# status-im/nim-blscurve

Hardware: AMD Instinct MI355X
Metric: BLS sig verifications/sec (batch) (higher is better)
Workload: dtype int64

## Files before the change

nim-blscurve_amd/csrc/host_api.inc:

```
#pragma once
#include "plan.hpp"
#include "devres.hpp"
using plan::SIG_SLOTS_MAX;
namespace cols = plan::cols;
static_assert(plan::WAVE == (uint32_t)WAVE && plan::N_LINES == (uint32_t)N_LINES, "plan.hpp restates the wave size and the Miller loop's step count");
static_assert(plan::FP_WORDS == (uint32_t)FPW && plan::G1_WORDS == (uint32_t)G1W && plan::G2_WORDS == (uint32_t)G2W && plan::F12_WORDS == (uint32_t)F12W,
              "plan.hpp restates the words of an element in device buffers");

struct msm_ws {
    dev_buf<uint8_t> d_pts, d_sc;
    dev_buf<uint32_t> pts_int;
    dev_buf<uint32_t> hist, offs, cursor, sorted, order, chist, winout, out, part, shist;
    dev_event ev_fork, ev_bucketed, ev_g[2], ev_tail[2];
    dev_buf<uint4> buckets, segout;
};
struct msm_many_ws {
    dev_buf<uint8_t> d_pts, d_sc;
    dev_buf<uint32_t> pts_int, offs_dev, hist, offs, cursor, order, chist, sorted, part, out;
    dev_buf<uint4> buckets, segout;
};
struct ptab_ws {
    dev_buf<uint32_t> scratch, hist, offs, cursor, order, chist, sorted, part, out;
    dev_buf<uint4> buckets, segout;
    uint32_t last_plan[3] = {0, 0, 0};
// ... 517 lines not shown
    }
    if (hi > B) hi = (uint32_t)B;
    size_t base = n_total / B, rem = n_total % B;
    auto off = [&](size_t c) { return c < rem ? (base + 1) * c : base * c + rem; };
    *first = off(lo);
    *count = off(hi) - off(lo);
}

static void host_sha256_32(const uint32_t (&in)[8], uint32_t (&out)[8]) {
    uint32_t w[16] = {in[0], in[1], in[2], in[3], in[4], in[5], in[6], in[7], 0x80000000u, 0, 0, 0, 0, 0, 0, 256};
    sha256_init(out);
    sha256_compress_core(out, w);
}
static void host_serial_chain(const uint8_t rnd[32], size_t n, uint64_t* out) {
    uint32_t seed[8], nx[8];
    for (int i = 0; i < 8; i++) nx[i] = ((uint32_t)rnd[4 * i] << 24) | ((uint32_t)rnd[4 * i + 1] << 16) | ((uint32_t)rnd[4 * i + 2] << 8) | rnd[4 * i + 3];
    host_sha256_32(nx, seed);
    for (size_t j = 0; j < n; j++) {
        uint64_t r;
        do {
            host_sha256_32(seed, nx);
            for (int i = 0; i < 8; i++) seed[i] = nx[i];
            r = digest_low_u64_le(seed);
        } while (r == 0);
        out[j] = r;
    }
}
static void host_combine_chain(const uint8_t rnd[32], size_t n, uint64_t* out) {
    uint32_t seed[8], nx[8];
    for (int i = 0; i < 8; i++) seed[i] = ((uint32_t)rnd[4 * i] << 24) | ((uint32_t)rnd[4 * i + 1] << 16) | ((uint32_t)rnd[4 * i + 2] << 8) | rnd[4 * i + 3];
    int avail = 0;
    for (size_t i = 0; i < n; i++) {
        for (;;) {
            if (avail == 0) {
                host_sha256_32(seed, nx);
                for (int j = 0; j < 8; j++) seed[j] = nx[j];
                avail = 4;
            }
            avail--;
            uint64_t w = (uint64_t)bswap32(seed[2 * avail]) | ((uint64_t)bswap32(seed[2 * avail + 1]) << 32);
            if (w != 0) {
                out[i] = w;
                break;
            }
        }
    }
}

static inline void launch_k_tail(const mi355_bls_ctx* c, hipStream_t st, const uint32_t* L, uint32_t* states, uint32_t kk, int mode, uint32_t* gt_out,
                                 uint32_t* verdict, uint32_t sstride, int blob) {
    if (c->coop) k_tail_rows<<<1, K_TAIL_THREADS, 0, st>>>(L, states, kk, mode, gt_out, verdict, sstride, blob);
    else k_tail<<<1, TAIL_THREADS, 0, st>>>(L, states, kk, mode, gt_out, verdict, sstride, blob);
}
static void launch_lines_at(const pair_store& ps, const plan::stage& t, uint32_t first, uint32_t count, hipStream_t st) {
    if (!t.team) {
        k_lines<<<t.grid, WAVE, 0, st>>>(ps.P, ps.H, first, count, ps.stride, ps.lines);
        return;
    }
    switch (t.form) {
        case plan::TEAM_ROWS: k_team_lines_rows<<<t.grid, 256, 0, st>>>(ps.P, ps.H, first, count, ps.stride, ps.lines); break;
        case plan::TEAM_ROWS2: k_team_lines_rows2<<<t.grid, 256, 0, st>>>(ps.P, ps.H, first, count, ps.stride, ps.lines); break;
        case plan::TEAM_SPREAD: k_team_lines_spread<<<t.grid, WAVE, 0, st>>>(ps.P, ps.H, first, count, ps.stride, ps.lines); break;
        case plan::TEAM_WIDE: k_team_lines<<<t.grid, WAVE, 0, st>>>(ps.P, ps.H, first, count, ps.stride, ps.lines); break;
    }
}
static void launch_lines(const pair_store& ps, const plan::lines_plan& p, hipStream_t st) {
    launch_lines_at(ps, p.main, 0, p.main_pairs, st);
    if (p.extra_pairs) launch_lines_at(ps, p.extra, p.main_pairs, p.extra_pairs, st);
}

static int enqueue_line_products(mi355_bls_ctx* c, const pair_store& ps, uint32_t npairs, hipStream_t st, hipEvent_t mid_ev) {
    c->fold_form = (c->coop || c->alone) ? 1 : 0;
    const plan::lineprod_plan p = plan::lineprod_for(c->slots, c->nblk_cap, ps.stride, npairs, c->fold_form != 0);
    k_lineprod<<<dim3(N_LINES, p.nblk), WAVE, 0, st>>>(ps.lines, npairs, ps.stride, p.m, c->d_lpart, p.nblk, p.per_lane);
    if (mid_ev) HIPCHK(hipEventRecord(mid_ev, st));
    if (c->fold_form) {
        uint32_t* mid = c->d_lpart + plan::lpart_mid_words(c->nblk_cap);
        k_fold<<<dim3(N_LINES, p.nb1), TAIL_THREADS, 0, st>>>(c->d_lpart, p.nblk * WAVE, p.per, p.live - (p.nb1 - 1) * p.per, p.nb1 > 1 ? mid : c->d_L);
        if (p.nb1 > 1) k_fold<<<dim3(N_LINES, 1), TAIL_THREADS, 0, st>>>(mid, p.nb1, p.nb1, p.nb1, c->d_L);
    } else {
        k_lineprod2<<<N_LINES, WAVE, 0, st>>>(c->d_lpart, p.nblk * WAVE, c->d_L);
    }
    return 0;
}

static int run_pairs(mi355_bls_ctx* c, const uint8_t* d_sets, size_t n, hipStream_t st, bool pop = false);
static int run_slice(mi355_bls_ctx* c, mi355_bls_ctx* p, const uint8_t* d_sets, size_t n_total, uint32_t nchunks, uint32_t chunk_lo, uint32_t chunk_cnt,
                     size_t tuple_base, size_t n, int serial, size_t serial_off, uint32_t slice, hipStream_t st, hipEvent_t blind_done, bool pop = false) {
    HIPCHK(hipEventRecord(c->ev[0], st));
    if (serial) {
        HIPCHK(hipMemcpyAsync(c->d_r, p->h_r.data() + serial_off, n * 8, hipMemcpyHostToDevice, st));
    } else {
        k_blind<<<plan::waves_for(chunk_cnt), WAVE, 0, st>>>(p->d_rnd, n_total, nchunks, chunk_lo, chunk_cnt, tuple_base, n, p->d_carry + 8 * (slice & 1),
                                                                p->d_carry + 8 * ((slice + 1) & 1), c->d_r);
    }
    if (blind_done) HIPCHK(hipEventRecord(blind_done, st));
    return run_pairs(c, d_sets, n, st, pop);
}
static int run_pairs(mi355_bls_ctx* c, const uint8_t* d_sets, size_t n, hipStream_t st, bool pop) {
    const uint32_t n32 = (uint32_t)n;
    const pair_store ps = c->batch_pairs();
    HIPCHK(hipEventRecord(c->ev[1], st));
    const plan::slice_plan p = plan::slice_for(c->slots, c->coop, c->coop && ensure_side(c), n);
    const uint32_t nb = p.nb, cw = p.cw, nwin = p.nwin, total = p.total;
    const bool fork = p.side == plan::SIDE_FORK, fork_sig = p.side == plan::SIDE_FORK_SIG;
    const auto stream_of = [&](plan::stream_role r) { return r == plan::STREAM_CALLER ? st : r == plan::STREAM_SIDE2 && c->side2 ? c->side2 : c->side; };
    hipStream_t sd = stream_of(p.pk_stream);
    hipStream_t ss = stream_of(p.sig_stream);
    if (fork || fork_sig) HIPCHK(hipStreamWaitEvent(c->side, c->ev[1], 0));
    if (fork && sd != c->side) HIPCHK(hipStreamWaitEvent(sd, c->ev[1], 0));
    launch_hash_map(c, d_sets, n32, st, pop);
    HIPCHK(hipEventRecord(c->ev_hm, st));
    launch_hash_clear(c, ps, n32, st);
    HIPCHK(hipEventRecord(c->ev[2], st));
    if (p.pkmul_spread) k_pkmul_spread<<<nb, WAVE, 0, sd>>>(d_sets, n32, c->d_r, ps.P, ps.stride, c->d_flags, c->d_pktab);
    else k_pkmul<<<nb, WAVE, 0, sd>>>(d_sets, n32, c->d_r, ps.P, ps.stride, c->d_flags, c->d_pktab);
    HIPCHK(hipEventRecord(c->ev[3], sd));
    {
        msm_win W{nwin, cw, 0};
        uint32_t *hist = c->d_sig_hist, *offs = hist + SIG_SLOTS_MAX, *cursor = offs + SIG_SLOTS_MAX;
        HIPCHK(hipEventRecord(c->ev_s0, ss));
        HIPCHK(hipMemsetAsync(hist, 0, (size_t)total * 4, ss));
        k_sig_convert<<<nb, WAVE, 0, ss>>>(d_sets, n32, c->d_sig_pts);
        k_msm_hist<<<dim3(nb, nwin), WAVE, 0, ss>>>(reinterpret_cast<const uint8_t*>(c->d_r.p), 8, n32, W, cw, hist);
        k_msm_scan<<<nwin, WAVE, 0, ss>>>(hist, cw, offs, cursor);
        k_msm_scatter<<<dim3(nb, nwin), WAVE, 0, ss>>>(reinterpret_cast<const uint8_t*>(c->d_r.p), 8, n32, W, cw, cursor, c->d_sig_sorted);
        k_sig_bucket<<<p.bucket_grid, WAVE, 0, ss>>>(c->d_sig_pts, c->d_sig_sorted, offs, hist, n32, cw, p.lshift, total,
                                                     c->d_sig_consts + (cw == 8 ? (size_t)SIG_SLOTS_MAX * G1W : 0), ps.H, ps.P, ps.stride, (size_t)n32);
        c->sig_c = cw;
        c->sig_slots = total;
        c->agg_valid = false;
    }
    uint32_t npairs = n32 + total;
    if (p.extra_apart) launch_lines_at(ps, p.extra_lines, n32, total, ss);
    HIPCHK(hipEventRecord(c->ev[4], ss));
    if (fork) {
        HIPCHK(hipStreamWaitEvent(st, c->ev[4], 0));
        HIPCHK(hipStreamWaitEvent(st, c->ev[3], 0));
    }
    HIPCHK(hipEventRecord(c->ev_l0, st));
    launch_lines(ps, p.lines, st);
    if (fork_sig) HIPCHK(hipStreamWaitEvent(st, c->ev[4], 0));
    HIPCHK(hipEventRecord(c->ev[5], st));
    {
        int rcp = enqueue_line_products(c, ps, npairs, st, c->ev_lp);
        if (rcp) return rcp;
    }
    c->wide_recorded = true;
    HIPCHK(hipEventRecord(c->ev[6], st));
    launch_k_tail(c, st, c->d_L, c->d_states, 1, 1, c->d_gt, c->d_flags + 1, 144, 0);
    HIPCHK(hipEventRecord(c->ev[7], st));
    HIPCHK(hipGetLastError());
    c->last_n = n;
    c->have_gt = false;
    c->gt_is_fv = false;
    return 0;
}

static int ensure_lanes(mi355_bls_ctx* c, int want) {
    for (dev_event* e : {&c->ev_sl0, &c->ev_blind[0], &c->ev_blind[1], &c->ev_blind[2]})
        if (!*e)
            if (int rc = e->create(hipEventDisableTiming)) return rc;
    int have = 0;
    for (int k = 0; k < want && k < 2; k++) {
        if (c->lane[k]) {
            have = k + 1;
            continue;
        }
        mi355_bls_ctx* raw = nullptr;
        dev_stream s;
        dev_event e;
        if (mi355_bls_ctx_create(&raw, c->device, c->cap) != 0) raw = nullptr;
        std::unique_ptr<mi355_bls_ctx> x(raw);
        if (!x || !s.create() || e.create(hipEventDisableTiming) != 0) {
            x.reset();
            (void)hipGetLastError();
            (void)hipSetDevice(c->device);
            break;
        }
        x->is_lane = true;
        x->coop = false;
        c->lane_st[k] = std::move(s);
        c->lane_ev[k] = std::move(e);
        c->lane[k] = std::move(x);
        have = k + 1;
    }
    return have;
}
static int run_shard(mi355_bls_ctx* c, const uint8_t* src_dev, const uint8_t* src_host, size_t n_total, uint32_t nchunks, uint32_t chunk_lo, uint32_t chunk_cnt,
                     size_t tuple_base, size_t n, int serial, const uint8_t rnd[32], hipStream_t st, bool pop = false, const uint64_t* chosen_r = nullptr) {
    (void)chunk_lo; (void)chunk_cnt;
    HIPCHK(hipSetDevice(c->device));
    if (c->fail_next_enqueue) {
        c->fail_next_enqueue = false;
// ... 3755 lines not shown
```

nim-blscurve_amd/csrc/kernels.hip:

```cpp
#include <hip/hip_runtime.h>

#include <algorithm>
#include <atomic>
#include <chrono>
#include <cstdio>
#include <cstdlib>
#include <cstring>
#include <mutex>
#include <string>
#include <unordered_map>
#include <vector>

#include "../../include/blscurve_mi355x.h"
#include "deser.hpp"
#include "h2c.hpp"
#include "pairing.hpp"
#include "vereach.hpp"
#include "aggveach.hpp"
#include "aggsets.hpp"
#include "aggbits.hpp"
#include "combsets.hpp"
#include "manyeach.hpp"
#include "pairprod.hpp"
#include "bymsg.hpp"
// ... 748 lines not shown
#endif
}
__global__ void __launch_bounds__(256) __attribute__((amdgpu_waves_per_eu(1, 1)))
k_team_lines_rows(const uint4* __restrict__ P, const uint4* __restrict__ H, uint32_t first, uint32_t count, size_t stride, uint4* __restrict__ lines) {
    team_lines_rows_body(P, H, first, count, stride, lines);
}
__global__ void __launch_bounds__(256) __attribute__((amdgpu_waves_per_eu(2, 2)))
k_team_lines_rows2(const uint4* __restrict__ P, const uint4* __restrict__ H, uint32_t first, uint32_t count, size_t stride, uint4* __restrict__ lines) {
    team_lines_rows_body(P, H, first, count, stride, lines);
}

#if defined(__HIP_DEVICE_COMPILE__)
#include "../build/pkmul_asm.inc"
__device__ __forceinline__ uint32_t pkmul_asm(uint64_t r, uint8_t* table, uint32_t off16, uint4* P, uint32_t pstride16, uint32_t lds) {
    uint32_t flag;
    asm volatile(BLS_PKMUL_ASM_BODY : "=v"(flag) : "v"((uint32_t)r), "v"((uint32_t)(r >> 32)), "s"(table), "s"(0u), "v"(off16), "s"(P), "s"(pstride16), "s"(lds) : BLS_PKMUL_ASM_CLOBBERS);
    return flag;
}
#endif
__device__ __forceinline__ void pkmul_body(const uint8_t* __restrict__ sets, uint32_t n, const uint64_t* __restrict__ r, uint4* __restrict__ P,
                                           size_t stride, uint32_t* __restrict__ flags, uint8_t* __restrict__ table) {
    uint32_t i = blockIdx.x * blockDim.x + threadIdx.x;
    if (i >= n) return;
    const uint32_t* w = reinterpret_cast<const uint32_t*>(sets + (size_t)i * 320);
    g1_aff pk = ld_g1a_blst(w);
    const bool inf = aff_is_inf(pk);
    if (inf) atomicOr(flags, 1u);
#if defined(__HIP_DEVICE_COMPILE__)
    if (table) {
        __shared__ bls_u32x4 key_slot[BLS_LDS_SLOT];
        if (inf) {
            soa_st_g1(P, stride, i, jac_inf<fp>());
        } else {
            fp2_lds_put((bls_lds_u32x4*)key_slot, fp2{pk.x, pk.y});
            if (pkmul_asm(r[i], table, i * 16u, P, (uint32_t)(stride * 16), (uint32_t)(uintptr_t)(bls_lds_u32x4*)key_slot))
                soa_st_g1(P, stride, i, jac_mul_u64_w4_body(pk, r[i]));
        }
        return;
    }
#endif
    g1_jac q = jac_mul_u64_w4_body(pk, r[i]);
    soa_st_g1(P, stride, i, q);
}
__global__ void __launch_bounds__(WAVE, 2) k_pkmul(const uint8_t* __restrict__ sets, uint32_t n, const uint64_t* __restrict__ r, uint4* __restrict__ P,
                                                   size_t stride, uint32_t* __restrict__ flags, uint8_t* __restrict__ table) {
    pkmul_body(sets, n, r, P, stride, flags, table);
}
__global__ void __launch_bounds__(WAVE) __attribute__((amdgpu_waves_per_eu(1, 1)))
k_pkmul_spread(const uint8_t* __restrict__ sets, uint32_t n, const uint64_t* __restrict__ r, uint4* __restrict__ P, size_t stride, uint32_t* __restrict__ flags,
               uint8_t* __restrict__ table) {
    pkmul_body(sets, n, r, P, stride, flags, table);
}

#if defined(__HIP_DEVICE_COMPILE__)
#include "../build/lines_asm.inc"
__device__ __forceinline__ void lines_asm(uint4* lines, uint32_t stride16, uint32_t off16, uint32_t skip, uint32_t lds_a, uint32_t lds_b) {
    asm volatile(BLS_LINES_ASM_BODY : : "s"(lines), "s"(stride16), "v"(off16), "v"(skip), "s"(lds_a), "s"(lds_b) : BLS_LINES_ASM_CLOBBERS);
}
#endif
__global__ void __launch_bounds__(WAVE) k_lines(const uint4* __restrict__ P, const uint4* __restrict__ H, uint32_t first, uint32_t count, size_t stride,
                                                uint4* __restrict__ lines) {
    uint32_t i = blockIdx.x * blockDim.x + threadIdx.x;
    if (i >= count) return;
    i += first;
    g1_jac p = soa_ld_g1(P, stride, i);
    g2_jac q = soa_ld_g2(H, stride, i);
#if defined(__HIP_DEVICE_COMPILE__)
    if (stride * 16 * 24 < ((size_t)1 << 32)) {
        __shared__ bls_u32x4 hand_over[4 * BLS_LDS_SLOT];
        const bool skip = jac_is_inf(p) | jac_is_inf(q);
        if (skip) {
            const line_t one = line_one();
            for (int s = 0; s < N_LINES; s++) {
                uint4* b = lines + (size_t)s * 24 * stride;
                soa_st2(b, stride, 0, i, one.l0);
                soa_st2(b, stride, 2, i, one.l1);
                soa_st2(b, stride, 4, i, one.l2);
            }
        }
        const g1_pre pre = g1_precompute(p);
        g2_proj t = g2_to_proj(q);
        bls_lds_u32x4* ho = (bls_lds_u32x4*)hand_over;
        fp2_lds_put(ho, fp2_reduce(t.x));
        fp2_lds_put(ho + BLS_LDS_SLOT, fp2_reduce(t.y));
        fp2_lds_put(ho + 2 * BLS_LDS_SLOT, fp2_reduce(t.z));
        fp2_lds_put(ho + 3 * BLS_LDS_SLOT, fp2{pre.z3, pre.nxz3});
        fp2_lds_put((bls_lds_u32x4*)bls_xchg, fp2{pre.xz, pre.y});
        lines_asm(lines, (uint32_t)(stride * 16), i * 16u, skip ? 1u : 0u, (uint32_t)(uintptr_t)ho, (uint32_t)(uintptr_t)(bls_lds_u32x4*)bls_xchg);
        return;
    }
#endif
    miller_lines(p, q, [&](int s, const line_t& l) {
        uint4* b = lines + (size_t)s * 24 * stride;
        soa_st2(b, stride, 0, i, l.l0);
        soa_st2(b, stride, 2, i, l.l1);
        soa_st2(b, stride, 4, i, l.l2);
    });
}

#if defined(__HIP_DEVICE_COMPILE__)
#include "../build/lineprod_asm.inc"
__device__ __forceinline__ void lineprod_asm(const uint4* step_base, uint32_t stride16, uint32_t npairs, uint32_t first, uint32_t rounds, uint32_t* out,
                                             uint32_t lds_buf) {
    asm volatile(BLS_LINEPROD_ASM_BODY : : "s"(step_base), "s"(stride16), "s"(npairs), "s"(first), "s"(rounds), "s"(out), "s"(lds_buf) : BLS_LINEPROD_ASM_CLOBBERS);
}
#endif
__global__ void __launch_bounds__(WAVE) k_lineprod(const uint4* __restrict__ lines, uint32_t npairs, size_t stride, uint32_t m,
                                                   uint32_t* __restrict__ part, uint32_t nblk, int per_lane) {
    uint32_t s = blockIdx.x, b = blockIdx.y;
    const uint4* base = lines + (size_t)s * 24 * stride;
    size_t first = (size_t)b * WAVE * m;
#if defined(__HIP_DEVICE_COMPILE__)
    __shared__ bls_u32x4 line_slots[4 * BLS_LDS_SLOT];
#endif
#if defined(__HIP_DEVICE_COMPILE__)
    if (per_lane == 1) {
        uint32_t rounds = 0;
        if (first < npairs) {
            size_t left = (npairs - first + WAVE - 1) / WAVE;
            rounds = left < m ? (uint32_t)left : m;
        }
        lineprod_asm(base, (uint32_t)(stride * 16), npairs, (uint32_t)first, rounds, part + ((size_t)s * nblk + b) * WAVE * F12W,
                     (uint32_t)(uintptr_t)(bls_lds_u32x4*)line_slots);
        return;
    }
#endif
    auto ld_line = [&](size_t j0) {
        size_t i = j0 + threadIdx.x;
        bool v = i < npairs;
        size_t ia = v ? i : j0;
        line_t l{soa_ld2(base, stride, 0, ia), soa_ld2(base, stride, 2, ia), soa_ld2(base, stride, 4, ia)};
        return line_t{fp2_select(v, l.l0, fp2_one()), fp2_select(v, l.l1, fp2_zero()), fp2_select(v, l.l2, fp2_zero())};
    };
    fp12 f = fp12_one();
#if defined(__HIP_DEVICE_COMPILE__)
    line_ops_lds lops{(bls_lds_u32x4*)line_slots};
#else
    line_ops_lds lops{};
#endif
    if (first < npairs) {
        f = fp12_from_line(ld_line(first));
#pragma clang loop unroll(disable)
        for (uint32_t j = 1; j < m; j++) {
            size_t j0 = first + (size_t)j * WAVE;
            if (j0 >= npairs) break;
// ... 1090 lines not shown
}
__global__ void __launch_bounds__(WAVE) k_ptab_scatter(const uint8_t* __restrict__ sc, fixed_addr A, pip_win W, uint32_t* __restrict__ cursor, uint32_t* __restrict__ sorted) {
    const uint32_t p = blockIdx.x * WAVE + threadIdx.x, w = blockIdx.y;
    if (p >= A.pairs) return;
    const int32_t d = pipm_digit(sc, p, W, w);
    if (d) {
        const uint32_t j = fixed_owner(A, p);
        const uint32_t pos = atomicAdd(&cursor[fixed_bucket(A, j, w, (uint32_t)(d < 0 ? -d : d))], 1u);
        sorted[pos] = fixed_entry(A, w, fixed_point(A, p, j)) | (d < 0 ? 0x80000000u : 0u);
    }
}
__global__ void __launch_bounds__(WAVE) k_debug_ptab_rows(const uint32_t* __restrict__ tab, uint32_t n, uint32_t w0, uint32_t nw, uint32_t i0, uint32_t ni,
                                                          uint32_t* __restrict__ out) {
    const uint32_t t = blockIdx.x * WAVE + threadIdx.x;
    if (t >= nw * ni) return;
    const uint32_t w = w0 + t / ni, i = i0 + t % ni;
    const uint32_t* e = tab + ((size_t)w * n + i) * (2 * FPW);
    uint32_t* o = out + (size_t)t * 24;
    if (e[FP_N]) {
        for (int q = 0; q < 24; q++) o[q] = 0;
    } else {
        st_fp_blst(o, ld_fp_int(e));
        st_fp_blst(o + 12, ld_fp_int(e + FPW));
    }
}

__device__ __forceinline__ g1_jac ld_jac_blst(const uint32_t* w, const g1_jac*) { return ld_g1_blst(w); }
__device__ __forceinline__ g2_jac ld_jac_blst(const uint32_t* w, const g2_jac*) { return ld_g2_blst(w); }
template <class F>
__global__ void __launch_bounds__(WAVE) k_jac_sum_blst(const uint32_t* __restrict__ parts, uint32_t k, uint32_t stride, uint32_t* __restrict__ out) {
    jac<F> acc = jac_inf<F>();
    for (uint32_t j = threadIdx.x; j < k; j += WAVE) acc = padd(acc, ld_jac_blst(parts + (size_t)j * stride, (const jac<F>*)nullptr));
    int top = 32;
    while (top >= 1 && (uint32_t)top >= k) top >>= 1;
    for (int d = top; d >= 1; d >>= 1) {
        jac<F> o = shfl_down_struct(acc, d);
        acc = padd(acc, o);
    }
    if (threadIdx.x == 0) st_jac_blst(out, acc);
}

__global__ void __launch_bounds__(WAVE) k_sig_convert(const uint8_t* __restrict__ sets, uint32_t n, uint32_t* __restrict__ pts_int) {
    uint32_t i = blockIdx.x * WAVE + threadIdx.x;
    if (i >= n) return;
    g2_aff q = ld_g2a_blst(reinterpret_cast<const uint32_t*>(sets + (size_t)i * 320 + 128));
    uint32_t* o = pts_int + (size_t)i * 4 * FPW;
    st_fp_int(o, q.x.c0); st_fp_int(o + FPW, q.x.c1); st_fp_int(o + 2 * FPW, q.y.c0); st_fp_int(o + 3 * FPW, q.y.c1);
}
__global__ void __launch_bounds__(WAVE) k_sig_consts(uint32_t c, uint32_t total, uint32_t* __restrict__ out) {
    uint32_t g = blockIdx.x * WAVE + threadIdx.x;
    if (g >= total) return;
    uint64_t sc = (uint64_t)(g & ((1u << c) - 1u)) << (c * (g >> c));
    g1_aff ng{fp_from_const(k::G1_X), fp_from_const(k::G1_NEG_Y)};
    st_g1_int(out + (size_t)g * G1W, jac_mul_u64(ng, sc));
}
__global__ void __launch_bounds__(WAVE) k_sig_bucket(const uint32_t* __restrict__ pts, const uint32_t* __restrict__ sorted, const uint32_t* __restrict__ offs,
                                                     const uint32_t* __restrict__ hist, uint32_t n, uint32_t c, uint32_t lshift, uint32_t total,
                                                     const uint32_t* __restrict__ consts, uint4* __restrict__ H, uint4* __restrict__ P, size_t stride, size_t base) {
    uint32_t t = blockIdx.x * WAVE + threadIdx.x;
    uint32_t L = 1u << lshift, g = t >> lshift, s = t & (L - 1);
    xyzz<fp2> part = xyzz_inf<fp2>();
    if (g < total) {
        uint32_t w = g >> c, cnt = hist[g], off = offs[g];
        const uint32_t* srt = sorted + (size_t)w * n + off;
        for (uint32_t j = s; j < cnt; j += L) {
            const uint32_t* pw = pts + (size_t)srt[j] * (4 * FPW);
            g2_aff q{fp2{ld_fp_int(pw), ld_fp_int(pw + FPW)}, fp2{ld_fp_int(pw + 2 * FPW), ld_fp_int(pw + 3 * FPW)}};
            part = xyzz_add_aff(part, q);
        }
    }
    g2_jac acc = jac_from_xyzz(part);
    for (uint32_t d = L >> 1; d >= 1; d >>= 1) {
        g2_jac o = shfl_down_struct(acc, (int)d);
        acc = jac_add(acc, o);
    }
    if (g < total && s == 0) {
        soa_st_g2(H, stride, base + g, acc);
        soa_st_g1(P, stride, base + g, ld_g1_int(consts + (size_t)g * G1W));
    }
}
__global__ void __launch_bounds__(WAVE) k_sig_fold(const uint4* __restrict__ H, size_t stride, uint32_t n, uint32_t nwin, uint32_t c, uint32_t* __restrict__ agg_out) {
    __shared__ uint32_t wsum[32 * G2W];
    uint32_t w = threadIdx.x;
    if (w < nwin) {
        g2_jac S = jac_inf<fp2>(), T = jac_inf<fp2>();
        for (uint32_t d = (1u << c) - 1; d >= 1; d--) {
            S = jac_add(S, soa_ld_g2(H, stride, (size_t)n + ((w << c) | d)));
            T = jac_add(T, S);
        }
        st_g2_int(wsum + (size_t)w * G2W, T);
    }
    __syncthreads();
    if (threadIdx.x == 0) {
        g2_jac acc = ld_g2_int(wsum + (size_t)(nwin - 1) * G2W);
        for (uint32_t j = nwin - 1; j-- > 0;) {
            for (uint32_t i = 0; i < c; i++) acc = jac_dbl(acc);
            acc = jac_add(acc, ld_g2_int(wsum + (size_t)j * G2W));
        }
        st_g2_blst(agg_out, acc);
    }
}

__global__ void __launch_bounds__(WAVE) k_deser(const uint8_t* __restrict__ pks, const uint8_t* __restrict__ msgs, const uint8_t* __restrict__ sigs,
                                                uint32_t n, uint32_t dflags, uint8_t* __restrict__ sets, uint8_t* __restrict__ status,
                                                uint32_t* __restrict__ flags) {
    uint32_t i = blockIdx.x * WAVE + threadIdx.x;
    if (i >= n) return;
// ... 897 lines not shown
```

nim-blscurve_amd/csrc/pairing.hpp:

```cpp
#pragma once
#include "curve.hpp"
#include "tower.hpp"

namespace bls {

constexpr int N_LINES = 68;

struct g1_pre {
    fp z3, xz, nxz3, y;
};

BLS_HD g1_pre g1_precompute(const g1_jac& p) {
    fp z2 = fp_sqr(p.z);
    fp xz = fp_mul(p.x, p.z);
    return g1_pre{fp_mul(z2, p.z), xz, fp_neg(fp_carry(fp_add_nc(fp_dbl_nc(xz), xz))), p.y};
}

BLS_HD line_t line_one() { return line_t{fp2_one(), fp2_zero(), fp2_zero()}; }

using g2_proj = g2_jac;

BLS_HD g2_proj g2_to_proj(const g2_jac& q) {
    fp2 z2 = fp2_sqr(q.z);
    return g2_proj{fp2_mul(q.x, q.z), q.y, fp2_mul(z2, q.z)};
}

BLS_MID fp2 fp2_sqr_minus_12sqr(const fp2& a, const fp2& e) {
    const fp e4s = fp_dbl_nc(fp_carry(fp_dbl_nc(fp_add_nc(e.c0, e.c1))));
    const fp ed = fp_sub_pos(e.c0, e.c1);
    const fp e3d = fp_carry(fp_add_nc(fp_dbl_nc(ed), ed));
    const fp e8 = fp_dbl_nc(fp_carry(fp_dbl_nc(fp_dbl_nc(e.c0))));
    const fp e3 = fp_carry(fp_add_nc(fp_dbl_nc(e.c1), e.c1));
    return fp2{fp_dot2(fp_add_nc(a.c0, a.c1), fp_sub_nc(a.c0, a.c1), fp_neg(e4s), e3d), fp_dot2(fp_dbl_nc(a.c0), a.c1, fp_neg(e8), e3)};
}
template <class M>
BLS_MID line_t miller_dbl_step_m(g2_proj& t, const g1_pre& p, const M& m) {
    fp2 B = m.sqr(t.y);
    fp2 C = m.sqr(t.z);
    fp2 X2 = m.sqr(t.x);
    fp2 C4 = fp2_dbl_nc(fp2_carry(fp2_dbl_nc(fp2_mul_xi_nc(C))));
    fp2 E = fp2_reduce(fp2_add_nc(fp2_dbl_nc(C4), C4));
    fp2 F = fp2_add_nc(fp2_dbl_nc(E), E);
    fp2 H = fp2_carry(fp2_sub_nc(fp2_sub_nc(m.sqr(fp2_add(t.y, t.z)), B), C));
    fp2 XY2 = fp2_carry(fp2_sub_nc(fp2_sub_nc(m.sqr(fp2_add(t.x, t.y)), X2), B));
    fp2 x3 = m.mul(XY2, fp2_carry(fp2_sub_nc(B, F)));
    fp2 y3 = fp2_sqr_minus_12sqr(fp2_carry(fp2_add_nc(B, F)), E);
    fp2 z3 = fp2_carry(fp2_dbl_nc(fp2_dbl_nc(m.mul(B, H))));
    t = g2_proj{x3, y3, z3};
    fp2 BE = fp2_sub_nc(B, E);
    return line_t{fp2{m.mul(BE.c0, p.z3), m.mul(BE.c1, p.z3)}, fp2{m.mul(X2.c0, p.nxz3), m.mul(X2.c1, p.nxz3)}, fp2{m.mul(H.c0, p.y), m.mul(H.c1, p.y)}};
}
BLS_MID line_t miller_dbl_step(g2_proj& t, const g1_pre& p) { return miller_dbl_step_m(t, p, mul_shared{}); }

BLS_MID line_t miller_add_step(g2_proj& t, const g2_proj& q, const g1_pre& p) {
    fp2 Y1Z2 = fp2_mul(t.y, q.z), X1Z2 = fp2_mul(t.x, q.z), Z1Z2 = fp2_mul(t.z, q.z);
    fp2 u = fp2_sub(fp2_mul(q.y, t.z), Y1Z2);
    fp2 v = fp2_sub(fp2_mul(q.x, t.z), X1Z2);
    fp2 uu = fp2_sqr(u), vv = fp2_sqr(v);
    fp2 vvv = fp2_mul(v, vv);
    fp2 R = fp2_mul(vv, X1Z2);
    fp2 A = fp2_carry(fp2_sub_nc(fp2_sub_nc(fp2_mul(uu, Z1Z2), vvv), fp2_dbl_nc(R)));
    fp2 x3 = fp2_mul(v, A);
    fp2 y3 = fp2_reduce(fp2_sub_nc(fp2_mul(u, fp2_sub_nc(R, A)), fp2_mul(vvv, Y1Z2)));
    fp2 z3 = fp2_mul(vvv, Z1Z2);
    fp2 c0 = fp2_carry(fp2_sub_nc(fp2_mul(u, q.x), fp2_mul(v, q.y)));
    fp2 c1 = fp2_mul(u, q.z);
    fp2 c2 = fp2_mul(v, q.z);
    t = g2_proj{x3, y3, z3};
    return line_t{fp2_mul_fp(c0, p.z3), fp2_neg(fp2_mul_fp(c1, p.xz)), fp2_mul_fp(c2, p.y)};
}

template <class Sink>
BLS_HD void miller_lines(const g1_jac& pj, const g2_jac& qj, Sink&& sink) {
    bool skip = jac_is_inf(pj) | jac_is_inf(qj);
    g1_pre p = g1_precompute(pj);
    g2_proj q = g2_to_proj(qj);
    q = g2_proj{fp2_reduce(q.x), fp2_reduce(q.y), fp2_reduce(q.z)};
    g2_proj t = q;
    int s = 0;
    uint64_t rest = k::X_ABS & ~(1ull << 63);
    int pos = 63;
#pragma clang loop unroll(disable)
    while (pos > 0) {
        const int next = rest ? 63 - __builtin_clzll(rest) : 0;
        int n = pos - next;
#pragma clang loop unroll(disable)
        do {
            line_t l = miller_dbl_step(t, p);
            sink(s++, skip ? line_one() : l);
        } while (--n > 0);
        if (rest) {
            line_t a = miller_add_step(t, q, p);
            sink(s++, skip ? line_one() : a);
            rest &= ~(1ull << next);
        }
        pos = next;
    }
}

template <class Src>
BLS_HD fp12 miller_combine(Src&& src) {
    fp12 f = fp12_one();
    int s = 0;
    for (int bit = 62; bit >= 0; bit--) {
        f = fp12_sqr(f);
        f = fp12_mul(f, src(s++));
        if ((k::X_ABS >> bit) & 1) f = fp12_mul(f, src(s++));
    }
    return fp12_conj(f);
}

BLS_HDN fp12 fp12_cyc_exp_x(const fp12& a) {
    fp12 r = a;
    for (int bit = 62; bit >= 0; bit--) {
        r = fp12_sqr(r);
        if ((k::X_ABS >> bit) & 1) r = fp12_mul(r, a);
    }
    return fp12_conj(r);
}

BLS_HDN fp12 final_exp(const fp12& f) {
    fp12 t = fp12_mul(fp12_conj(f), fp12_inv(f));
    t = fp12_mul(fp12_frob2(t), t);
    fp12 a = fp12_mul(fp12_cyc_exp_x(t), fp12_conj(t));
    a = fp12_mul(fp12_cyc_exp_x(a), fp12_conj(a));
    fp12 b = fp12_mul(fp12_cyc_exp_x(a), fp12_frob(a));
    fp12 c = fp12_mul(fp12_mul(fp12_cyc_exp_x(fp12_cyc_exp_x(b)), fp12_frob2(b)), fp12_conj(b));
    return fp12_mul(c, fp12_mul(fp12_sqr(t), t));
}

}
```

nim-blscurve_amd/csrc/plan.hpp:

```cpp
#ifndef BLS_PLAN_HPP
#define BLS_PLAN_HPP
#include <cstddef>
#include <cstdint>

namespace plan {

constexpr uint32_t WAVE = 64;
constexpr uint32_t N_LINES = 68;
constexpr uint32_t FP_WORDS = 16;
constexpr uint32_t G1_WORDS = 3 * FP_WORDS, G2_WORDS = 6 * FP_WORDS, F12_WORDS = 12 * FP_WORDS;
constexpr uint32_t SIG_SLOTS_MAX = 2048;
static_assert(((64u / 8) << 8) == SIG_SLOTS_MAX, "the buckets of the 8-bit digits");
constexpr size_t SIG_WIDE_MIN = 40000;
constexpr uint32_t FORK_ITEMS_PER_SLOT = 16;

constexpr uint32_t TEAM_CLEAR_ITEMS_PER_SLOT = 11, TEAM_LINES_ITEMS_PER_SLOT = 18;
inline uint32_t team_clear_max(uint32_t slots) { return slots * TEAM_CLEAR_ITEMS_PER_SLOT; }
inline uint32_t team_lines_max(uint32_t slots) { return slots * TEAM_LINES_ITEMS_PER_SLOT; }

inline uint32_t waves_for(uint32_t count) { return (count + WAVE - 1) / WAVE; }
constexpr uint32_t GATHER_THREADS = 256;
inline uint32_t gather_blocks_for(size_t count) { return (uint32_t)((count + GATHER_THREADS - 1) / GATHER_THREADS); }

enum team_form { TEAM_ROWS, TEAM_ROWS2, TEAM_SPREAD, TEAM_WIDE };
// ... 19 lines not shown
enum hash_map_form { HASH_MAP_ROWS, HASH_MAP_SPREAD, HASH_MAP_PLAIN };
struct hash_map_plan {
    hash_map_form form;
    uint32_t grid;
};
inline hash_map_plan hash_map_for(uint32_t slots, bool coop, uint32_t n32) {
    const uint32_t waves = (2 * n32 + WAVE - 1) / WAVE;
    if (coop && (2 * n32 + 3) / 4 <= slots - slots / 8) return {HASH_MAP_ROWS, (2 * n32 + 3) / 4};
    if (coop && waves <= slots) return {HASH_MAP_SPREAD, waves};
    return {HASH_MAP_PLAIN, waves};
}

constexpr size_t POP_MAX_KEYS = (size_t)1 << 30;
constexpr uint32_t POP_RECORD_THREADS = 256;
inline uint32_t pop_records_grid(size_t n) { return (uint32_t)((n * 80 + POP_RECORD_THREADS - 1) / POP_RECORD_THREADS); }

constexpr uint8_t ADMIT_BAD_PROOF = 8;
inline size_t admit_survivors(const uint8_t* key_st, const uint8_t* proof_st, size_t n, uint32_t* list) {
    size_t m = 0;
    for (size_t i = 0; i < n; i++)
        if (key_st[i] == 0 && proof_st[i] == 0) list[m++] = (uint32_t)i;
    return m;
}
inline size_t admit_merge(const uint8_t* key_st, const uint8_t* proof_st, size_t n, const uint32_t* list, const uint8_t* verdicts, size_t m, uint8_t* status,
                          uint32_t* zero) {
    for (size_t i = 0; i < n; i++) status[i] = key_st[i] ? key_st[i] : proof_st[i];
    for (size_t j = 0; j < m; j++)
        if (verdicts[j] != 1) status[list[j]] = ADMIT_BAD_PROOF;
    size_t nz = 0;
    for (size_t i = 0; i < n; i++)
        if (status[i] != 0 && key_st[i] == 0) zero[nz++] = (uint32_t)i;
    return nz;
}

inline stage clear_for(uint32_t slots, bool coop, uint32_t n32) {
    return coop && n32 <= team_clear_max(slots) ? team_stage(slots, n32) : one_lane_stage(n32);
}

struct lines_plan {
    uint32_t main_pairs;
    stage main;
    uint32_t extra_pairs;
    stage extra;
};
inline lines_plan lines_for(uint32_t slots, bool coop, uint32_t npairs, uint32_t extra) {
    if (coop && npairs <= team_lines_max(slots)) return {npairs, team_stage(slots, npairs), 0, {}};
    if (coop && extra && extra < npairs && extra <= team_lines_max(slots) &&
        (npairs + WAVE - 1) / WAVE > slots * (((npairs - extra + WAVE - 1) / WAVE + slots - 1) / slots)) {
        const uint32_t main_pairs = npairs - extra;
        return {main_pairs, one_lane_stage(main_pairs), extra, team_stage(slots, extra)};
    }
    return {npairs, one_lane_stage(npairs), 0, {}};
}

enum side_mode { SIDE_NONE, SIDE_FORK, SIDE_FORK_SIG };
inline bool pkmul_spread_for(uint32_t slots, bool coop, uint32_t n) { return coop && waves_for(n) <= slots; }
enum stream_role { STREAM_CALLER, STREAM_SIDE, STREAM_SIDE2 };
struct slice_plan {
    uint32_t nb;
    hash_map_plan hash_map;
    stage clear;
    bool pkmul_spread;
    side_mode side;
    stream_role pk_stream, sig_stream;
    uint32_t cw, nwin, total;
    uint32_t lshift, bucket_grid;
    bool extra_apart;
    stage extra_lines;
    lines_plan lines;
};
inline slice_plan slice_for(uint32_t slots, bool coop, bool have_side, size_t n) {
    slice_plan p{};
    const uint32_t n32 = (uint32_t)n;
    p.nb = waves_for(n32);
    const bool fork = have_side && n32 <= FORK_ITEMS_PER_SLOT * slots;
    const bool fork_sig = !fork && have_side;
    p.side = fork ? SIDE_FORK : fork_sig ? SIDE_FORK_SIG : SIDE_NONE;
    p.pk_stream = fork ? STREAM_SIDE2 : STREAM_CALLER;
    p.sig_stream = (fork || fork_sig) ? STREAM_SIDE : STREAM_CALLER;
    p.hash_map = hash_map_for(slots, coop, n32);
    p.clear = clear_for(slots, coop, n32);
    p.pkmul_spread = pkmul_spread_for(slots, coop, n32);
    p.cw = n >= SIG_WIDE_MIN ? 8 : 4, p.nwin = 64 / p.cw, p.total = p.nwin << p.cw;
    uint32_t per = n32 >> p.cw, lshift = 0;
    const uint32_t per_lane_min = coop ? 16u : 64u;
    while (lshift < 6 && (per >> (lshift + 1)) >= per_lane_min) lshift++;
    while (lshift < 6 && ((p.total << (lshift + 1)) <= 16 * slots) && (per >> (lshift + 1)) >= 2) lshift++;
    p.lshift = lshift;
    p.bucket_grid = ((p.total << lshift) + WAVE - 1) / WAVE;
    p.extra_apart = fork_sig || (fork && p.total <= team_lines_max(slots));
    p.extra_lines = p.total <= team_lines_max(slots) ? team_stage(slots, p.total) : one_lane_stage(p.total);
    p.lines = p.extra_apart ? lines_for(slots, coop, n32, 0) : lines_for(slots, coop, n32 + p.total, p.total);
    return p;
}

struct lineprod_plan {
    uint32_t nblk, m;
    int per_lane;
    uint32_t live, per, nb1;
};
inline lineprod_plan lineprod_for(uint32_t slots, uint32_t nblk_cap, uint32_t stride, uint32_t npairs, bool fold) {
    lineprod_plan p{};
    uint32_t nblk = slots / N_LINES;
    if (nblk < 1) nblk = 1;
    if (nblk > nblk_cap) nblk = nblk_cap;
    uint32_t m = (npairs + WAVE * nblk - 1) / (WAVE * nblk);
    if (m < 1) m = 1;
    nblk = (npairs + WAVE * m - 1) / (WAVE * m);
    p.nblk = nblk, p.m = m;
    p.per_lane = (uint64_t)stride * 16 * 24 + (uint64_t)npairs * 16 < (1ull << 32) ? 1 : 2;
    if (fold) {
        size_t first_last = (size_t)(nblk - 1) * WAVE * m;
        p.live = (nblk - 1) * WAVE + (npairs - first_last < WAVE ? (uint32_t)(npairs - first_last) : WAVE);
        p.per = 1;
        while (p.per * p.per < p.live) p.per++;
        p.nb1 = (p.live + p.per - 1) / p.per;
    }
    return p;
}

constexpr uint32_t LINEPROD_RANGES_MAX = 64, FOLD_MID_ROOM = 64;
constexpr uint32_t SUM_G2_PARTS_MAX = 2048;
constexpr size_t SUM_PARTS_BYTES = 2048 * 2 * G1_WORDS * 4;
static_assert((size_t)SUM_G2_PARTS_MAX * G2_WORDS * 4 == SUM_PARTS_BYTES, "2048 G2 partials, or twice as many G1 ones");
struct ctx_sizes {
    size_t stride, mstride;
    uint32_t nblk_cap;
    size_t lpart_words, lpart_mid_words;
    size_t export_bytes;
};
inline size_t lpart_mid_words(uint32_t nblk_cap) { return (size_t)N_LINES * nblk_cap * WAVE * F12_WORDS; }
inline ctx_sizes ctx_for(uint32_t slots, size_t max_sets) {
    ctx_sizes s{};
    s.stride = ((max_sets + 1 + SIG_SLOTS_MAX + WAVE - 1) / WAVE) * WAVE;
    s.mstride = ((2 * max_sets + WAVE - 1) / WAVE) * WAVE;
    const size_t nwaves = s.stride / WAVE;
    uint32_t nblk = slots / N_LINES;
    if (nblk < 1) nblk = 1;
    if (nblk > LINEPROD_RANGES_MAX) nblk = LINEPROD_RANGES_MAX;
    if (nblk > nwaves) nblk = (uint32_t)nwaves;
    s.nblk_cap = nblk;
    s.lpart_words = (size_t)N_LINES * (nblk * (WAVE + 1) + FOLD_MID_ROOM) * F12_WORDS;
    s.lpart_mid_words = lpart_mid_words(nblk);
    s.export_bytes = s.stride * 288 + SUM_PARTS_BYTES;
    return s;
// ... 729 lines not shown
    size_t pairs = len(j0);
    while (s.j1 < k && s.j1 - j0 < P.msms_max && len(s.j1) <= MSM_MANY_PAIRS_MAX && pairs + len(s.j1) <= MSM_MANY_PAIRS_MAX) pairs += len(s.j1++);
    const uint32_t kp = (uint32_t)(s.j1 - j0);
    s.pairs = (uint32_t)pairs;
    s.points = offsets ? s.pairs : (uint32_t)npoints;
    s.nv = kp * P.W.nwin;
    s.total = kp * P.buckets_per_msm;
    s.nseg = s.nv * P.segs_per_win;
    s.pair_grid = waves_for(s.pairs);
    s.order_grid = (s.total + WAVE * MSM_ORD_PER - 1) / (WAVE * MSM_ORD_PER);
    s.bucket_grid = waves_for(s.total);
    s.team = P.g2 ? 1 : ((size_t)s.nseg * 4 <= MSM_TEAM_LANES_MAX ? 4 : ((size_t)s.nseg * 2 <= MSM_TEAM_LANES_MAX ? 2 : 1));
    s.segred_grid = waves_for(s.nseg * s.team);
    return s;
}
struct msm_many_sizes {
    size_t pts_int;
    size_t offs_dev;
    size_t hist;
    size_t chist;
    size_t sorted;
    size_t buckets, segout;
    size_t part;
};
inline msm_many_sizes msm_many_extents(const msm_many_plan& P, const msm_many_pass& s) {
    msm_many_sizes z{};
    if (s.single || s.pairs == 0) return z;
    const size_t jac = P.g2 ? G2_WORDS : G1_WORDS;
    z.pts_int = (size_t)s.points * (jac / 3 * 2) * 4;
    z.offs_dev = P.shared ? 0 : (s.j1 - s.j0 + 1) * 4;
    z.hist = (size_t)s.total * 4;
    z.chist = 256 * 4;
    z.sorted = (size_t)s.pairs * P.W.nwin * 4;
    z.buckets = (size_t)s.total * jac * 4;
    z.segout = (size_t)s.nseg * jac * 4;
    z.part = (size_t)s.nv * P.nsplit * jac * 4;
    return z;
}
inline msm_many_sizes msm_many_sizes_for(const msm_many_plan& P, const size_t* offsets, size_t npoints, size_t k) {
    msm_many_sizes m{};
    const auto up = [](size_t& a, size_t b) { a = a < b ? b : a; };
    for (size_t j = 0; j < k;) {
        const msm_many_pass s = msm_many_next(P, offsets, npoints, k, j);
        const msm_many_sizes z = msm_many_extents(P, s);
        up(m.pts_int, z.pts_int), up(m.offs_dev, z.offs_dev), up(m.hist, z.hist), up(m.chist, z.chist), up(m.sorted, z.sorted), up(m.buckets, z.buckets),
            up(m.segout, z.segout), up(m.part, z.part);
        j = s.j1;
    }
    return m;
}

constexpr uint32_t TOAFF_DEVICE_LANES = 256 * 4 * WAVE;
constexpr uint32_t TOAFF_RUN_MAX = 8;
constexpr uint32_t TOAFF_CHUNK_POINTS = 1u << 24;
static_assert((uint64_t)TOAFF_CHUNK_POINTS * 288 < (1ull << 33) && TOAFF_CHUNK_POINTS % TOAFF_RUN_MAX == 0, "a chunk's byte offsets are size_t; whole runs per chunk");
struct to_affine_plan {
    uint32_t run;
    uint32_t chunk;
};
struct to_affine_launch {
    size_t first;
    uint32_t n;
    uint32_t lanes, grid;
};
inline to_affine_plan to_affine_for(size_t n, uint32_t force_run = 0) {
    to_affine_plan p{};
    size_t run = force_run ? force_run : (n + TOAFF_DEVICE_LANES - 1) / TOAFF_DEVICE_LANES;
    p.run = (uint32_t)(run < 1 ? 1 : (run > TOAFF_RUN_MAX ? TOAFF_RUN_MAX : run));
    p.chunk = TOAFF_CHUNK_POINTS;
    return p;
}
inline to_affine_launch to_affine_next(const to_affine_plan& p, size_t n, size_t first) {
    to_affine_launch l{};
    l.first = first;
    l.n = (uint32_t)(n - first < p.chunk ? n - first : p.chunk);
    l.lanes = (l.n + p.run - 1) / p.run;
    l.grid = waves_for(l.lanes);
    return l;
}

constexpr uint32_t FIXED_WBITS_MIN = 5, FIXED_WBITS_MAX = 16;
constexpr uint64_t FIXED_ENTRIES_MAX = 1ull << 31;
constexpr size_t FIXED_ENTRY_BYTES = 2 * FP_WORDS * 4;
constexpr uint32_t FIXED_PAIRS_MAX = MSM_MANY_PAIRS_MAX;
constexpr size_t FIXED_SCRATCH_BYTES = (size_t)256 << 20;
inline uint32_t fixed_nwin(size_t wbits, size_t nbits) { return (uint32_t)((nbits + 1 + wbits - 1) / wbits); }
constexpr size_t FIXED_WBITS_WIDE_FROM = (size_t)1 << 14;
inline uint32_t fixed_wbits_for(size_t npoints) { return npoints < FIXED_WBITS_WIDE_FROM ? 8 : 16; }
inline bool fixed_args_ok(size_t npoints, size_t wbits, size_t nbits) {
    if (npoints == 0 || nbits == 0 || nbits > 256 || (wbits != 0 && (wbits < FIXED_WBITS_MIN || wbits > FIXED_WBITS_MAX))) return false;
    if (npoints > FIXED_ENTRIES_MAX) return false;
    const uint64_t W = fixed_nwin(wbits ? wbits : fixed_wbits_for(npoints), nbits);
    return W * (uint64_t)npoints <= FIXED_ENTRIES_MAX;
}
inline size_t fixed_table_bytes(size_t npoints, size_t wbits, size_t nbits) {
    if (!fixed_args_ok(npoints, wbits, nbits)) return 0;
    return (size_t)fixed_nwin(wbits ? wbits : fixed_wbits_for(npoints), nbits) * npoints * FIXED_ENTRY_BYTES;
}
inline pip_win fixed_win(size_t wbits, size_t nbits) {
    pip_win W{};
    W.nbits = (uint32_t)nbits;
    W.nwin = fixed_nwin(wbits, nbits);
    W.wbase = (uint32_t)wbits, W.wrem = 0;
    W.cbk = (uint32_t)wbits - 1;
    for (uint32_t w = 0; w + 1 < W.nwin; w++) {
        const uint32_t bit = w * W.wbase + W.wbase - 1;
// ... 212 lines not shown
```

nim-blscurve_amd/csrc/toaffine.hpp:

```cpp
#pragma once
#include "curve.hpp"
#include "plan.hpp"

namespace bls {

BLS_HD fp f_inv(const fp& a) { return fp_inv(fp_reduce(a)); }
BLS_HD fp2 f_inv(const fp2& a) { return fp2_inv(fp2_reduce(a)); }

template <class F, class Load, class Store, class StoreInf>
BLS_HD void to_affine_run(uint32_t count, Load&& load, Store&& store, StoreInf&& store_inf) {
    F pre[plan::TOAFF_RUN_MAX];
    F acc = f_one<F>();
    bool any = false;
#pragma clang loop unroll(disable)
    for (uint32_t i = 0; i < count; i++) {
        const F z = load(i).z;
        if (!f_is_zero(z)) {
            acc = f_mul(acc, z);
            any = true;
        }
        pre[i] = acc;
    }
    F inv = any ? f_inv(acc) : f_zero<F>();
#pragma clang loop unroll(disable)
    for (uint32_t i = count; i-- > 0;) {
        const jac<F> p = load(i);
        if (f_is_zero(p.z)) {
            store_inf(i);
            continue;
        }
        const F zi = i ? f_mul(inv, pre[i - 1]) : inv;
        inv = f_mul(inv, p.z);
        const F zi2 = f_sqr(zi);
        store(i, aff<F>{f_mul(p.x, zi2), f_mul(p.y, f_mul(zi2, zi))});
    }
}

}
```

Baseline: 6.077 million.

## Normalise G1 points to affine before Miller line generation to drop Z multiplies

Result: slower. 5.994 million (-1.4%).

```diff
diff --git a/nim-blscurve_amd/csrc/host_api.inc b/nim-blscurve_amd/csrc/host_api.inc
--- a/nim-blscurve_amd/csrc/host_api.inc
+++ b/nim-blscurve_amd/csrc/host_api.inc
@@ -593,8 +593,14 @@
     if (c->coop) k_tail_rows<<<1, K_TAIL_THREADS, 0, st>>>(L, states, kk, mode, gt_out, verdict, sstride, blob);
     else k_tail<<<1, TAIL_THREADS, 0, st>>>(L, states, kk, mode, gt_out, verdict, sstride, blob);
 }
-static void launch_lines_at(const pair_store& ps, const plan::stage& t, uint32_t first, uint32_t count, hipStream_t st) {
+static void enqueue_g1_normalise(const pair_store& ps, uint32_t first, uint32_t count, hipStream_t st) {
+    if (!count) return;
+    const plan::g1norm_plan g = plan::g1norm_for(count);
+    k_g1_normalise<<<g.grid, WAVE, 0, st>>>(ps.P, first, count, ps.stride, g.run, g.lanes);
+}
+static void launch_lines_at(const pair_store& ps, const plan::stage& t, uint32_t first, uint32_t count, hipStream_t st, bool p_affine = false) {
     if (!t.team) {
+        if (!p_affine) enqueue_g1_normalise(ps, first, count, st);
         k_lines<<<t.grid, WAVE, 0, st>>>(ps.P, ps.H, first, count, ps.stride, ps.lines);
         return;
     }
@@ -605,8 +611,8 @@
         case plan::TEAM_WIDE: k_team_lines<<<t.grid, WAVE, 0, st>>>(ps.P, ps.H, first, count, ps.stride, ps.lines); break;
     }
 }
-static void launch_lines(const pair_store& ps, const plan::lines_plan& p, hipStream_t st) {
-    launch_lines_at(ps, p.main, 0, p.main_pairs, st);
+static void launch_lines(const pair_store& ps, const plan::lines_plan& p, hipStream_t st, bool p_affine = false) {
+    launch_lines_at(ps, p.main, 0, p.main_pairs, st, p_affine);
     if (p.extra_pairs) launch_lines_at(ps, p.extra, p.main_pairs, p.extra_pairs, st);
 }
 
@@ -656,6 +662,7 @@
     HIPCHK(hipEventRecord(c->ev[2], st));
     if (p.pkmul_spread) k_pkmul_spread<<<nb, WAVE, 0, sd>>>(d_sets, n32, c->d_r, ps.P, ps.stride, c->d_flags, c->d_pktab);
     else k_pkmul<<<nb, WAVE, 0, sd>>>(d_sets, n32, c->d_r, ps.P, ps.stride, c->d_flags, c->d_pktab);
+    if (p.pk_affine) enqueue_g1_normalise(ps, 0, n32, sd);
     HIPCHK(hipEventRecord(c->ev[3], sd));
     {
         msm_win W{nwin, cw, 0};
@@ -673,14 +680,14 @@
         c->agg_valid = false;
     }
     uint32_t npairs = n32 + total;
-    if (p.extra_apart) launch_lines_at(ps, p.extra_lines, n32, total, ss);
+    if (p.extra_apart) launch_lines_at(ps, p.extra_lines, n32, total, ss, true);
     HIPCHK(hipEventRecord(c->ev[4], ss));
     if (fork) {
         HIPCHK(hipStreamWaitEvent(st, c->ev[4], 0));
         HIPCHK(hipStreamWaitEvent(st, c->ev[3], 0));
     }
     HIPCHK(hipEventRecord(c->ev_l0, st));
-    launch_lines(ps, p.lines, st);
+    launch_lines(ps, p.lines, st, p.pk_affine);
     if (fork_sig) HIPCHK(hipStreamWaitEvent(st, c->ev[4], 0));
     HIPCHK(hipEventRecord(c->ev[5], st));
     {
diff --git a/nim-blscurve_amd/csrc/kernels.hip b/nim-blscurve_amd/csrc/kernels.hip
--- a/nim-blscurve_amd/csrc/kernels.hip
+++ b/nim-blscurve_amd/csrc/kernels.hip
@@ -824,6 +824,14 @@
     pkmul_body(sets, n, r, P, stride, flags, table);
 }
 
+__global__ void __launch_bounds__(WAVE) k_g1_normalise(uint4* __restrict__ P, uint32_t first, uint32_t count, size_t stride, uint32_t run, uint32_t lanes) {
+    const uint32_t lane = blockIdx.x * WAVE + threadIdx.x;
+    if (run == 0 || run > plan::G1NORM_RUN) return;
+    g1_normalise_run(
+        plan::g1norm_lane_points(run, lanes, count, lane), [&](uint32_t i) { return soa_ld_g1(P, stride, first + plan::g1norm_point(lanes, lane, i)); },
+        [&](uint32_t i, const g1_jac& a) { soa_st_g1(P, stride, first + plan::g1norm_point(lanes, lane, i), a); });
+}
+
 #if defined(__HIP_DEVICE_COMPILE__)
 #include "../build/lines_asm.inc"
 __device__ __forceinline__ void lines_asm(uint4* lines, uint32_t stride16, uint32_t off16, uint32_t skip, uint32_t lds_a, uint32_t lds_b) {
@@ -850,19 +858,19 @@
                 soa_st2(b, stride, 4, i, one.l2);
             }
         }
-        const g1_pre pre = g1_precompute(p);
+        const g1_pre pre = g1_precompute_aff(p);
         g2_proj t = g2_to_proj(q);
         bls_lds_u32x4* ho = (bls_lds_u32x4*)hand_over;
         fp2_lds_put(ho, fp2_reduce(t.x));
         fp2_lds_put(ho + BLS_LDS_SLOT, fp2_reduce(t.y));
         fp2_lds_put(ho + 2 * BLS_LDS_SLOT, fp2_reduce(t.z));
-        fp2_lds_put(ho + 3 * BLS_LDS_SLOT, fp2{pre.z3, pre.nxz3});
-        fp2_lds_put((bls_lds_u32x4*)bls_xchg, fp2{pre.xz, pre.y});
+        fp2_lds_put(ho + 3 * BLS_LDS_SLOT, fp2{pre.xz, pre.nxz3});
+        fp2_lds_put((bls_lds_u32x4*)bls_xchg, fp2{pre.y, pre.y});
         lines_asm(lines, (uint32_t)(stride * 16), i * 16u, skip ? 1u : 0u, (uint32_t)(uintptr_t)ho, (uint32_t)(uintptr_t)(bls_lds_u32x4*)bls_xchg);
         return;
     }
 #endif
-    miller_lines(p, q, [&](int s, const line_t& l) {
+    miller_lines<true>(p, q, [&](int s, const line_t& l) {
         uint4* b = lines + (size_t)s * 24 * stride;
         soa_st2(b, stride, 0, i, l.l0);
         soa_st2(b, stride, 2, i, l.l1);
@@ -2059,7 +2067,12 @@
     if (g >= total) return;
     uint64_t sc = (uint64_t)(g & ((1u << c) - 1u)) << (c * (g >> c));
     g1_aff ng{fp_from_const(k::G1_X), fp_from_const(k::G1_NEG_Y)};
-    st_g1_int(out + (size_t)g * G1W, jac_mul_u64(ng, sc));
+    g1_jac j = jac_mul_u64(ng, sc);
+    if (!jac_is_inf(j)) {
+        const fp zi = f_inv(j.z), zi2 = fp_sqr(zi);
+        j = g1_jac{fp_mul(j.x, zi2), fp_mul(j.y, fp_mul(zi2, zi)), fp_one()};
+    }
+    st_g1_int(out + (size_t)g * G1W, j);
 }
 __global__ void __launch_bounds__(WAVE) k_sig_bucket(const uint32_t* __restrict__ pts, const uint32_t* __restrict__ sorted, const uint32_t* __restrict__ offs,
                                                      const uint32_t* __restrict__ hist, uint32_t n, uint32_t c, uint32_t lshift, uint32_t total,
diff --git a/nim-blscurve_amd/csrc/pairing.hpp b/nim-blscurve_amd/csrc/pairing.hpp
--- a/nim-blscurve_amd/csrc/pairing.hpp
+++ b/nim-blscurve_amd/csrc/pairing.hpp
@@ -16,6 +16,8 @@
     return g1_pre{fp_mul(z2, p.z), xz, fp_neg(fp_carry(fp_add_nc(fp_dbl_nc(xz), xz))), p.y};
 }
 
+BLS_HD g1_pre g1_precompute_aff(const g1_jac& p) { return g1_pre{fp_one(), p.x, fp_neg(fp_carry(fp_add_nc(fp_dbl_nc(p.x), p.x))), p.y}; }
+
 BLS_HD line_t line_one() { return line_t{fp2_one(), fp2_zero(), fp2_zero()}; }
 
 using g2_proj = g2_jac;
@@ -33,7 +35,7 @@
     const fp e3 = fp_carry(fp_add_nc(fp_dbl_nc(e.c1), e.c1));
     return fp2{fp_dot2(fp_add_nc(a.c0, a.c1), fp_sub_nc(a.c0, a.c1), fp_neg(e4s), e3d), fp_dot2(fp_dbl_nc(a.c0), a.c1, fp_neg(e8), e3)};
 }
-template <class M>
+template <bool AFF = false, class M>
 BLS_MID line_t miller_dbl_step_m(g2_proj& t, const g1_pre& p, const M& m) {
     fp2 B = m.sqr(t.y);
     fp2 C = m.sqr(t.z);
@@ -48,11 +50,16 @@
     fp2 z3 = fp2_carry(fp2_dbl_nc(fp2_dbl_nc(m.mul(B, H))));
     t = g2_proj{x3, y3, z3};
     fp2 BE = fp2_sub_nc(B, E);
-    return line_t{fp2{m.mul(BE.c0, p.z3), m.mul(BE.c1, p.z3)}, fp2{m.mul(X2.c0, p.nxz3), m.mul(X2.c1, p.nxz3)}, fp2{m.mul(H.c0, p.y), m.mul(H.c1, p.y)}};
+    fp2 l0;
+    if constexpr (AFF) l0 = fp2_reduce(BE);
+    else l0 = fp2{m.mul(BE.c0, p.z3), m.mul(BE.c1, p.z3)};
+    return line_t{l0, fp2{m.mul(X2.c0, p.nxz3), m.mul(X2.c1, p.nxz3)}, fp2{m.mul(H.c0, p.y), m.mul(H.c1, p.y)}};
 }
 BLS_MID line_t miller_dbl_step(g2_proj& t, const g1_pre& p) { return miller_dbl_step_m(t, p, mul_shared{}); }
+BLS_MID line_t miller_dbl_step_aff(g2_proj& t, const g1_pre& p) { return miller_dbl_step_m<true>(t, p, mul_shared{}); }
 
-BLS_MID line_t miller_add_step(g2_proj& t, const g2_proj& q, const g1_pre& p) {
+template <bool AFF = false>
+BLS_MID line_t miller_add_step_m(g2_proj& t, const g2_proj& q, const g1_pre& p) {
     fp2 Y1Z2 = fp2_mul(t.y, q.z), X1Z2 = fp2_mul(t.x, q.z), Z1Z2 = fp2_mul(t.z, q.z);
     fp2 u = fp2_sub(fp2_mul(q.y, t.z), Y1Z2);
     fp2 v = fp2_sub(fp2_mul(q.x, t.z), X1Z2);
@@ -63,17 +70,21 @@
     fp2 x3 = fp2_mul(v, A);
     fp2 y3 = fp2_reduce(fp2_sub_nc(fp2_mul(u, fp2_sub_nc(R, A)), fp2_mul(vvv, Y1Z2)));
     fp2 z3 = fp2_mul(vvv, Z1Z2);
-    fp2 c0 = fp2_carry(fp2_sub_nc(fp2_mul(u, q.x), fp2_mul(v, q.y)));
+    fp2 c0 = fp2_sub_nc(fp2_mul(u, q.x), fp2_mul(v, q.y));
+    if constexpr (AFF) c0 = fp2_reduce(c0);
+    else c0 = fp2_mul_fp(fp2_carry(c0), p.z3);
     fp2 c1 = fp2_mul(u, q.z);
     fp2 c2 = fp2_mul(v, q.z);
     t = g2_proj{x3, y3, z3};
-    return line_t{fp2_mul_fp(c0, p.z3), fp2_neg(fp2_mul_fp(c1, p.xz)), fp2_mul_fp(c2, p.y)};
+    return line_t{c0, fp2_neg(fp2_mul_fp(c1, p.xz)), fp2_mul_fp(c2, p.y)};
 }
+BLS_MID line_t miller_add_step(g2_proj& t, const g2_proj& q, const g1_pre& p) { return miller_add_step_m<false>(t, q, p); }
+BLS_MID line_t miller_add_step_aff(g2_proj& t, const g2_proj& q, const g1_pre& p) { return miller_add_step_m<true>(t, q, p); }
 
-template <class Sink>
+template <bool AFF = false, class Sink>
 BLS_HD void miller_lines(const g1_jac& pj, const g2_jac& qj, Sink&& sink) {
     bool skip = jac_is_inf(pj) | jac_is_inf(qj);
-    g1_pre p = g1_precompute(pj);
+    g1_pre p = AFF ? g1_precompute_aff(pj) : g1_precompute(pj);
     g2_proj q = g2_to_proj(qj);
     q = g2_proj{fp2_reduce(q.x), fp2_reduce(q.y), fp2_reduce(q.z)};
     g2_proj t = q;
@@ -86,11 +97,11 @@
         int n = pos - next;
 #pragma clang loop unroll(disable)
         do {
-            line_t l = miller_dbl_step(t, p);
+            line_t l = AFF ? miller_dbl_step_aff(t, p) : miller_dbl_step(t, p);
             sink(s++, skip ? line_one() : l);
         } while (--n > 0);
         if (rest) {
-            line_t a = miller_add_step(t, q, p);
+            line_t a = AFF ? miller_add_step_aff(t, q, p) : miller_add_step(t, q, p);
             sink(s++, skip ? line_one() : a);
             rest &= ~(1ull << next);
         }
diff --git a/nim-blscurve_amd/csrc/plan.hpp b/nim-blscurve_amd/csrc/plan.hpp
--- a/nim-blscurve_amd/csrc/plan.hpp
+++ b/nim-blscurve_amd/csrc/plan.hpp
@@ -95,6 +95,26 @@
     }
     return {npairs, one_lane_stage(npairs), 0, {}};
 }
+
+constexpr uint32_t G1NORM_RUN = 8;
+struct g1norm_plan {
+    uint32_t run;
+    uint32_t lanes, grid;
+};
+inline g1norm_plan g1norm_for(uint32_t count) {
+    g1norm_plan g{};
+    const uint32_t run = (count + WAVE - 1) / WAVE;
+    g.run = run < 1 ? 1 : (run > G1NORM_RUN ? G1NORM_RUN : run);
+    g.lanes = (count + g.run - 1) / g.run;
+    g.grid = waves_for(g.lanes);
+    return g;
+}
+constexpr uint32_t g1norm_lane_points(uint32_t run, uint32_t lanes, uint32_t count, uint32_t lane) {
+    if (lane >= lanes || lane >= count) return 0;
+    const uint32_t mine = (count - lane + lanes - 1) / lanes;
+    return mine < run ? mine : run;
+}
+constexpr size_t g1norm_point(uint32_t lanes, uint32_t lane, uint32_t i) { return lane + (size_t)i * lanes; }
 
 enum side_mode { SIDE_NONE, SIDE_FORK, SIDE_FORK_SIG };
 inline bool pkmul_spread_for(uint32_t slots, bool coop, uint32_t n) { return coop && waves_for(n) <= slots; }
@@ -111,6 +131,7 @@
     bool extra_apart;
     stage extra_lines;
     lines_plan lines;
+    bool pk_affine;
 };
 inline slice_plan slice_for(uint32_t slots, bool coop, bool have_side, size_t n) {
     slice_plan p{};
@@ -134,6 +155,7 @@
     p.extra_apart = fork_sig || (fork && p.total <= team_lines_max(slots));
     p.extra_lines = p.total <= team_lines_max(slots) ? team_stage(slots, p.total) : one_lane_stage(p.total);
     p.lines = p.extra_apart ? lines_for(slots, coop, n32, 0) : lines_for(slots, coop, n32 + p.total, p.total);
+    p.pk_affine = !p.lines.main.team;
     return p;
 }
 
@@ -969,6 +991,7 @@
 
 constexpr uint32_t TOAFF_DEVICE_LANES = 256 * 4 * WAVE;
 constexpr uint32_t TOAFF_RUN_MAX = 8;
+static_assert(G1NORM_RUN <= TOAFF_RUN_MAX, "k_g1_normalise runs to_affine_run: a lane's points fit its prefix array");
 constexpr uint32_t TOAFF_CHUNK_POINTS = 1u << 24;
 static_assert((uint64_t)TOAFF_CHUNK_POINTS * 288 < (1ull << 33) && TOAFF_CHUNK_POINTS % TOAFF_RUN_MAX == 0, "a chunk's byte offsets are size_t; whole runs per chunk");
 struct to_affine_plan {
diff --git a/nim-blscurve_amd/csrc/toaffine.hpp b/nim-blscurve_amd/csrc/toaffine.hpp
--- a/nim-blscurve_amd/csrc/toaffine.hpp
+++ b/nim-blscurve_amd/csrc/toaffine.hpp
@@ -36,4 +36,10 @@
     }
 }
 
+template <class Load, class Store>
+BLS_HD void g1_normalise_run(uint32_t count, Load&& load, Store&& store) {
+    to_affine_run<fp>(
+        count, load, [&](uint32_t i, const g1_aff& a) { store(i, g1_jac{a.x, a.y, fp_one()}); }, [](uint32_t) {});
 }
+
+}
```
